# WagnerGroup/pyqmc

Measured on AMD Instinct MI355X. Metric: walker-steps/sec (VMC sweep, 64e- Slater-Jastrow), higher is better.
Workload: dtype f64

## Files before the change

pyqmc_amd/csrc/pqa_capi.hip:

```cpp
#include "pqa_internal.hpp"

static thread_local std::string g_create_error;


static int member_masks(pqa_handle* h, const pqa_system_t* sys, PbcDev& P) {
  P.memb_mask = nullptr;
  P.memb_E = 0;
  const int side = 2 * sys->member_M + 1, E = side, T = side + 2 * E, nc = sys->n_member_class, nj = std::min(sys->nL, 128);
  if ((size_t)nc * T * T * T * 16 > ((size_t)64 << 20)) return 0;
  std::vector<unsigned char> mem((size_t)nc * side * side * side);
  std::vector<int> imgn((size_t)sys->nL * 3);
  HIPCHK(hipMemcpy(mem.data(), sys->member, mem.size(), hipMemcpyDefault));
  HIPCHK(hipMemcpy(imgn.data(), sys->img_n, imgn.size() * sizeof(int), hipMemcpyDefault));
  for (int j = 0; j < nj; ++j)
    for (int c = 0; c < 3; ++c)
      if (std::abs(imgn[3 * j + c]) > E) return 0;
  std::vector<unsigned long long> mask((size_t)nc * T * T * T * 2, 0ull);
  for (int cl = 0; cl < nc; ++cl)
    for (int i0 = 0; i0 < T; ++i0)
      for (int i1 = 0; i1 < T; ++i1)
        for (int i2 = 0; i2 < T; ++i2) {
          unsigned long long* m = &mask[2 * ((((size_t)cl * T + i0) * T + i1) * T + i2)];
          for (int j = 0; j < nj; ++j) {
            const int n0 = i0 - E + imgn[3 * j], n1 = i1 - E + imgn[3 * j + 1], n2 = i2 - E + imgn[3 * j + 2];
// ... 697 lines not shown
        }
        rc2[k] = rc * rc;
      }
      TRY(upload_table(h, rc2.data(), rc2.size(), &tmp_d)); S.ecp_rc2 = tmp_d;
    }
  }
  {
    std::vector<double> quad, quadw;
    ecp_quadrature_tables(quad, quadw);
    TRY(upload_table(h, quad.data(), quad.size(), &h->d_quad));
    TRY(upload_table(h, quadw.data(), quadw.size(), &h->d_quadw));
    std::vector<int> na((size_t)std::max(h->necp, 1), 0), qo((size_t)std::max(h->necp, 1), 0);
    h->ecp_nch.assign((size_t)h->necp, 0);
    for (int k = 0; k < h->necp; ++k) {
      h->ecp_nch[k] = sys->ecp_chan_off[k + 1] - sys->ecp_chan_off[k];
      na[k] = h->ecp_nch[k] <= 2 ? 6 : 12;
      qo[k] = ecp_quadrature_offset(na[k]);
    }
    TRY(upload_table(h, na.data(), na.size(), &h->d_ecp_naip));
    TRY(upload_table(h, qo.data(), qo.size(), &h->d_ecp_qoff));
    S.ecp_naip = h->d_ecp_naip; S.ecp_qoff = h->d_ecp_qoff;
    S.ecp_naip_max = 0;
    for (int k = 0; k < h->necp; ++k) S.ecp_naip_max = std::max(S.ecp_naip_max, na[k]);
  }
  {
    std::vector<int> ptk, pti;
    for (int k = 0; k < h->necp; ++k) {
      const int nch = sys->ecp_chan_off[k + 1] - sys->ecp_chan_off[k];
      const int naip = nch <= 2 ? 6 : 12;
      for (int i = 0; i < naip; ++i) { ptk.push_back(k); pti.push_back(i); }
    }
    h->tm_P = (int)ptk.size();
    TRY(upload_table(h, ptk.data(), ptk.size(), &h->d_ptk));
    TRY(upload_table(h, pti.data(), pti.size(), &h->d_pti));
  }
  return 0;
}

extern "C" int pqa_create(const pqa_system_t* sys, int device, pqa_handle_t** out) {
  *out = nullptr;
  pqa_handle* h = new pqa_handle();
  h->device = device;
  int rc = create_impl(h, sys);
  if (rc) {
    g_create_error = h->err;
    pqa_destroy(h);
    return rc;
  }
  *out = h;
  return 0;
}

extern "C" void pqa_destroy(pqa_handle_t* h) {
  if (!h) return;
  (void)hipSetDevice(h->device);
  if (h->stream) (void)hipStreamSynchronize(h->stream);
  for (void* p : h->owned) (void)hipFree(p);
  DevBuf* bufs[] = {&h->b_x, &h->b_T[0], &h->b_T[1], &h->b_dsign[0], &h->b_dsign[1], &h->b_dlog[0], &h->b_dlog[1],
                    &h->b_cache[0], &h->b_cache[1], &h->b_aval, &h->b_bval, &h->b_pts, &h->b_motmp, &h->b_out, &h->b_widx,
                    &h->b_mask, &h->b_ao, &h->b_flag, &h->b_newpos, &h->b_aux, &h->b_accept, &h->b_accrec, &h->b_acccnt, &h->b_accw,
                    &h->b_gauss, &h->b_unif, &h->b_kc, &h->b_en, &h->b_means, &h->b_sign, &h->b_log, &h->b_ju, &h->b_rot,
                    &h->b_eunif, &h->b_elocal, &h->b_ecnt, &h->b_eoff, &h->b_epts[0], &h->b_epts[1], &h->b_ewgt[0],
                    &h->b_ewgt[1], &h->b_epte[0], &h->b_epte[1], &h->b_emo[0], &h->b_emo[1], &h->b_ecp, &h->b_xt, &h->b_Tt[0], &h->b_Tt[1], &h->b_rc[0], &h->b_rc[1], &h->b_sel[0], &h->b_sel[1], &h->b_auxt, &h->b_kpart, &h->b_rbuf, &h->b_vbuf, &h->b_act, &h->b_alt_x, &h->b_alt_T[0], &h->b_alt_T[1], &h->b_alt_dsign[0], &h->b_alt_dsign[1], &h->b_alt_dlog[0], &h->b_alt_dlog[1], &h->b_alt_cache[0], &h->b_alt_cache[1], &h->b_alt_aval, &h->b_alt_bval, &h->b_alt_j3u, &h->b_rsidx, &h->b_tpos, &h->b_twgt, &h->b_tlive, &h->b_trat, &h->b_tmcnt, &h->b_tmoff, &h->b_tmpass, &h->b_tmamp, &h->b_tmacc, &h->b_tmidx, &h->b_tmapos, &h->b_tmu, &h->b_tmtile, &h->b_tmaoff, &h->b_tmptw, &h->b_tmmarks, &h->b_dmcw, &h->b_dmcold, &h->b_dmcr2, &h->b_dmcout, &h->b_j3u, &h->b_dwrap, &h->b_wrap, &h->b_epass, &h->b_eptw[0], &h->b_eptw[1], &h->b_econ[0], &h->b_econ[1], &h->b_eu0[0], &h->b_eu0[1], &h->b_tves, &h->b_pgdet, &h->b_pbcd0, &h->b_pbcmask, &h->b_pbcth, &h->b_tmuold, &h->b_gauss_b, &h->b_unif_b, &h->b_orbphi[0], &h->b_orbphi[1], &h->b_s2out, &h->b_symx, &h->b_symdet[0], &h->b_symdet[1], &h->b_symout, &h->b_sqq, &h->b_sqout, &h->b_sqpart, &h->b_sqacc, &h->b_e2tab, &h->b_e2out, &h->b_e2acc};
  for (DevBuf* b : bufs)
    if (b->p) (void)hipFree(b->p);
  for (auto& d : h->dm)
    for (DevBuf* b : {&d.pos, &d.row, &d.f, &d.newpos, &d.keep_pos, &d.keep_row, &d.keep_f, &d.cfg})
      if (b->p) (void)hipFree(b->p);
  for (DevBuf* b : {&h->dm_val, &h->dm_norm[0], &h->dm_norm[1], &h->dm_tmp, &h->dm_ijkl, &h->dm_assign[0], &h->dm_assign[1], &h->dm_ratio, &h->dm_acc})
    if (b->p) (void)hipFree(b->p);
  for (auto& pr : h->prof_events) { (void)hipEventDestroy(pr.first); (void)hipEventDestroy(pr.second); }
  for (auto& pr : h->prof2_events) { (void)hipEventDestroy(pr.first); (void)hipEventDestroy(pr.second); }
  for (auto& pr : h->prof3_events) { (void)hipEventDestroy(pr.first); (void)hipEventDestroy(pr.second); }
  if (h->ev0) (void)hipEventDestroy(h->ev0);
  if (h->ev1) (void)hipEventDestroy(h->ev1);
  if (h->pin_tot) (void)hipHostFree(h->pin_tot);
  if (h->b_ovl.p) (void)hipFree(h->b_ovl.p);
  if (h->pin_ovl) (void)hipHostFree(h->pin_ovl);
  if (h->en_stream) { (void)hipStreamSynchronize(h->en_stream); (void)hipStreamDestroy(h->en_stream); }
  if (h->draw_stream) { (void)hipStreamSynchronize(h->draw_stream); (void)hipStreamDestroy(h->draw_stream); }
  for (hipEvent_t e : h->draw_ev) if (e) (void)hipEventDestroy(e);
  for (hipEvent_t e : h->en_ev)
    if (e) (void)hipEventDestroy(e);
  if (h->stream) (void)hipStreamDestroy(h->stream);
  delete h;
}
// ... 98 lines not shown
  } else
    FAIL("unknown parameter name");
  h->saved_valid = false;
  return 0;
}

extern "C" int pqa_get_param(pqa_handle_t* h, const char* name, double* out, int64_t n) {
  HIPCHK(hipSetDevice(h->device));
  HIPCHK(hipStreamSynchronize(h->stream));
  const std::string k(name);
  const double* src = nullptr;
  int64_t want = 0;
  if (k == "acoeff") { src = h->d_acoeff; want = (int64_t)h->natom * h->na * 2; }
  else if (k == "bcoeff") { src = h->d_bcoeff; want = (int64_t)h->nb * 3; }
  else if (k == "det_coeff") { src = h->d_detcoeff; want = h->ndet; }
  else if (k == "mo_coeff_alpha") { src = h->d_mo[0]; want = (int64_t)h->nao * h->nmo[0]; }
  else if (k == "mo_coeff_beta") { src = h->d_mo[1]; want = (int64_t)h->nao * h->nmo[1]; }
  else if (k == "radial_table_info") {
    if (n != 2) FAIL("parameter size mismatch");
    long used = 0;
    for (size_t q = 0; q + 1 < h->rt_shells.size(); q += 2)
      if (h->rt_shells[q] >= 0) used = std::max(used, (long)h->rt_shells[q] + (long)h->rt_shells[q + 1] * PQA_RT_REC);
    out[0] = (double)used; out[1] = h->rt_err;
    return 0;
  }
  else FAIL("unknown parameter name");
  if (n != want) FAIL("parameter size mismatch");
  HIPCHK(hipMemcpy(out, src, n * sizeof(double), hipMemcpyDefault));
  return 0;
}


extern "C" int pqa_eval_ao(pqa_handle_t* h, const double* pts, int64_t npts, int ncomp, double* out) {
  HIPCHK(hipSetDevice(h->device));
  if (!h->has_slater) FAIL("handle has no orbital tables");
  if (ncomp != 1 && ncomp != 4 && ncomp != 5) FAIL("ncomp must be 1, 4 or 5");
  if (h->twist) FAIL("AO-only evaluation is not available for twisted cells (complex AOs); use pqa_eval_mo");
  if (npts <= 0) return 0;
  const size_t nout = (size_t)ncomp * npts * h->nao;
  TRY(ensure(h, h->b_pts, (size_t)npts * 3 * sizeof(double)));
  TRY(ensure(h, h->b_ao, nout * sizeof(double)));
  TRY(copy_in(h, h->b_pts.p, pts, (size_t)npts * 3 * sizeof(double)));
  const dim3 grid((unsigned)((npts + 63) / 64)), block(64);
  TRY(launch_ao(h, plain_points((const double*)h->b_pts.p, npts), npts, ncomp, (double*)h->b_ao.p));
  TRY(check_launch(h, "k_ao"));
  return copy_out(h, out, h->b_ao.p, nout * sizeof(double));
// ... 1046 lines not shown
  if (launches) *launches = h->prof3_launches;
  if (total_ms) *total_ms = h->prof3_ms;
  if (groups) {
    LwCtx lc;
    TRY(lw_setup(h, false, lc));
    *groups = lc.Gm;
  }
  return 0;
}
extern "C" int pqa_set_ecp_naip(pqa_handle_t* h, int32_t naip) {
  HIPCHK(hipSetDevice(h->device));
  if (naip != 0 && ecp_quadrature_offset(naip) < 0) FAIL("naip must be one of 6, 12, 18, 26, 32, 50 (eval_ecp.py:266-267), or 0 for the per-atom default");
  if (h->necp == 0) { h->ecp_naip = naip; return 0; }
  std::vector<int> na((size_t)h->necp), qo((size_t)h->necp);
  for (int k = 0; k < h->necp; ++k) {
    na[k] = naip ? naip : (h->ecp_nch[k] <= 2 ? 6 : 12);
    qo[k] = ecp_quadrature_offset(na[k]);
  }
  HIPCHK(hipStreamSynchronize(h->stream));
  h->ecp_hint_valid = false; h->last_ecp_dev[0] = h->last_ecp_dev[1] = nullptr;
  if (h->last_ecp_points < 0) h->last_ecp_points = 0;
  h->S.ecp_naip_max = 0;
  for (int k = 0; k < h->necp; ++k) h->S.ecp_naip_max = std::max(h->S.ecp_naip_max, na[k]);
  HIPCHK(hipMemcpy(h->d_ecp_naip, na.data(), na.size() * sizeof(int), hipMemcpyHostToDevice));
  HIPCHK(hipMemcpy(h->d_ecp_qoff, qo.data(), qo.size() * sizeof(int), hipMemcpyHostToDevice));
  h->ecp_naip = naip;
  return 0;
}
extern "C" int pqa_last_ecp_points(pqa_handle_t* h, int64_t* npoints) {
  if (h->last_ecp_points < 0 && h->last_ecp_dev[0]) {
    HIPCHK(hipSetDevice(h->device));
    long t[2];
    TRY(copy_in(h, &t[0], h->last_ecp_dev[0], sizeof(long)));
    TRY(copy_out(h, &t[1], h->last_ecp_dev[1], sizeof(long)));
    h->last_ecp_points = t[0] + t[1];
  }
  *npoints = h->last_ecp_points;
  return 0;
}
```

pyqmc_amd/csrc/pqa_ecp.hpp:

```cpp
#pragma once
#include "pqa_energy.hpp"
#include "pqa_lw.hpp"

#define PQA_ECP_WB 4

struct EcpTab {
  const int* ecp_chan_off;
  const int* ecp_term_off;
  const int* ecp_term_n;
  const double* ecp_term_exp;
  const double* ecp_term_coef;
  const double* atom;
  const int* naip;
  const int* qoff;
};

__host__ __device__ inline size_t ecp_tab_bytes(int necp, int nchan, int nterm) {
  const size_t d = (size_t)4 * necp + 2 * (size_t)nterm, i = (size_t)(necp + 1) + (nchan + 1) + nterm + 2 * (size_t)necp;
  return d * sizeof(double) + ((i + 1) / 2) * 2 * sizeof(int);
}

__device__ __forceinline__ EcpTab ecp_stage(const SysDev& S, int nchan, int nterm, double* lds, int tid, int nthreads) {
  double* atom = lds;
  double* ex = atom + 4 * S.necp;
// ... 207 lines not shown
          const double* qd = B.quad + 3 * (qoff + ip);
          const double vx = Rm[0] * qd[0] + Rm[1] * qd[1] + Rm[2] * qd[2];
          const double vy = Rm[3] * qd[0] + Rm[4] * qd[1] + Rm[5] * qd[2];
          const double vz = Rm[6] * qd[0] + Rm[7] * qd[1] + Rm[8] * qd[2];
          const double rix = r * vx, riy = r * vy, riz = r * vz;
          const double cosv = (dx * rix + dy * riy + dz * riz) / (r * sqrt(rix * rix + riy * riy + riz * riz));
          double wsum = 0.0;
          for (int c = 0; c < nch - 1; ++c) wsum += (v[c] / prob) * (2 * c + 1) * legendre_l(c, cosv);
          const long slot = off + ip;
          B.pts[s][3 * slot] = (x0 - dx) + rix;
          B.pts[s][3 * slot + 1] = (y0 - dy) + riy;
          B.pts[s][3 * slot + 2] = (z0 - dz) + riz;
          B.wgt[s][slot] = wsum * B.quadw[qoff + ip];
          B.pte[s][slot] = e;
          B.ptw[s][slot] = (int)w;
          B.u0[s][slot] = U0;
        }
    }
    __builtin_amdgcn_fence(__ATOMIC_ACQ_REL, "wavefront");
    __builtin_amdgcn_wave_barrier();
  }
}

template <bool PBC, bool CX = false>
static __global__ __launch_bounds__(256) void k_ecp_point_lw(SysDev S, LwState L, EcpBuf B, int s, int has_slater, int has_jastrow,
                                                      const double* __restrict__ mo, long npts, long W, double* __restrict__ contrib,
                                                      const double* __restrict__ mo1 = nullptr, long npts1 = 0, double* __restrict__ contrib1 = nullptr) {
  if (blockIdx.y) { s = 1; mo = mo1; npts = npts1; contrib = contrib1; }
  const long p = (long)blockIdx.x * 256 + threadIdx.x;
  if (p >= npts || (B.ptot[s] && p >= *B.ptot[s])) return;
  const int e = B.pte[s][p];
  const long w = B.ptw[s][p];
  const int n = s ? S.ndn : S.nup, i = e - s * S.nup, nmo = S.nmo[s];
  double ratio = 1.0, ratio_im = 0.0;
  if (has_slater) {
    const double* row = mo + (size_t)p * nmo;
    if (CX) {
      const double* Ti = L.Tt[s] + (size_t)i * 2 * n * W + w;
      const int* occ = S.det_occ[s];
      const int nh = nmo / 2;
      double rr = 0.0, ri = 0.0;
      const bool lines = S.occ_ident[s] && ((n | nh) & 7) == 0;
      for (int k0 = 0; k0 < n; k0 += 8) {
        double tr[8], ti[8], a[8], b[8];
#pragma unroll
        for (int u = 0; u < 8; ++u) {
          const int k = (k0 + u < n) ? k0 + u : n - 1;
          tr[u] = Ti[(size_t)(2 * k) * W]; ti[u] = Ti[(size_t)(2 * k + 1) * W];
        }
        if (lines) {
          const double4 al = *reinterpret_cast<const double4*>(row + k0), ah = *reinterpret_cast<const double4*>(row + k0 + 4);
          const double4 bl = *reinterpret_cast<const double4*>(row + nh + k0), bh = *reinterpret_cast<const double4*>(row + nh + k0 + 4);
          a[0] = al.x; a[1] = al.y; a[2] = al.z; a[3] = al.w; a[4] = ah.x; a[5] = ah.y; a[6] = ah.z; a[7] = ah.w;
          b[0] = bl.x; b[1] = bl.y; b[2] = bl.z; b[3] = bl.w; b[4] = bh.x; b[5] = bh.y; b[6] = bh.z; b[7] = bh.w;
        } else {
#pragma unroll
          for (int u = 0; u < 8; ++u) {
            const int o = occ[(k0 + u < n) ? k0 + u : n - 1];
// ... 18 lines not shown
        for (int u = 0; u < 16; ++u) t[u] = Ti[(size_t)(k0 + u) * W];
#pragma unroll
        for (int u = 0; u < 4; ++u) {
          r += q[u].x * t[4 * u]; r += q[u].y * t[4 * u + 1]; r += q[u].z * t[4 * u + 2]; r += q[u].w * t[4 * u + 3];
        }
      }
    } else {
      const int* occ = S.det_occ[s];
      for (int k = 0; k < n; ++k) r += row[occ[k]] * Ti[(size_t)k * W];
    }
    ratio = r;
    }
  }
  if (has_jastrow) {
    double U, g[3], lp, ee, ei;
    if (S.jq_on) jas_eval_lane_m<0, PBC, true, true>(S, L.xt, W, w, e, B.pts[s][3 * p], B.pts[s][3 * p + 1], B.pts[s][3 * p + 2], 1, 0, 1, U, g, lp, ee, ei, -1, true);
    else jas_eval_lane<0, PBC>(S, L.xt, W, w, e, B.pts[s][3 * p], B.pts[s][3 * p + 1], B.pts[s][3 * p + 2], 1, 0, 1, U, g, lp, ee, ei);
    const double ej = exp(U - B.u0[s][p]);
    ratio *= ej; ratio_im *= ej;
  }
  contrib[p] = ratio * B.wgt[s][p];
  if (CX) contrib[npts + p] = ratio_im * B.wgt[s][p];
}
```

pyqmc_amd/csrc/pqa_energy.hip:

```cpp
#include "pqa_internal.hpp"

int energy_dev(pqa_handle* h, double threshold, const double* rot, const double* unif, uint64_t seed, uint32_t step,
               bool soa_current, bool aos_T_needed, bool assemble) {
  const long W = h->W;
  struct JsxOnce { pqa_handle* h; ~JsxOnce() { h->jsx_current = false; } } jsx_once{h};
  if (!soa_current) h->jsx_current = false;
  bool soa_T = false;
  struct Side { pqa_handle* h = nullptr; hipStream_t main = nullptr; ~Side() { if (h) h->stream = main; } } side;
  bool side_join = false;
  TRY(ensure(h, h->b_kc, (size_t)4 * W * sizeof(double)));
  TRY(ensure(h, h->b_en, (size_t)(h->cplx ? 7 : 6) * W * sizeof(double)));
  const bool will_defer = h->necp > 0 && h->ecpb_on == 0 && h->ecp_defer != 0 && !h->S.pbc && h->ecp_hint_valid && (h->ecp_evals % 16) != 0 &&
                          (W * (long)h->N * h->necp * std::max(h->S.ecp_naip_max, 1)) * (long)(64 + 8 * std::max(h->nmo[0], h->nmo[1])) <= (long)256 << 20;
  auto side_begin = [&]() -> int {
    if (!h->en_stream) {
      HIPCHK(hipStreamCreateWithFlags(&h->en_stream, hipStreamNonBlocking));
      for (hipEvent_t& e : h->en_ev) HIPCHK(hipEventCreateWithFlags(&e, hipEventDisableTiming));
    }
    HIPCHK(hipEventRecord(h->en_ev[0], h->stream));
    HIPCHK(hipStreamWaitEvent(h->en_stream, h->en_ev[0], 0));
    side.main = h->stream; side.h = h;
    h->stream = h->en_stream;
    return 0;
  };
// ... 50 lines not shown
    hipLaunchKernelGGL((k_ewald<>), dim3((unsigned)W), dim3(PQA_EWALD_T), lds_ew, h->stream, h->S, h->ew, x,
                       soa ? 1L : (long)h->N * 3, soa ? 3 * W : 3L, soa ? W : 1L, W, (double*)h->b_kc.p);
    TRY(check_launch(h, "k_ewald"));
  }
  if (side.h) {
    HIPCHK(hipEventRecord(h->en_ev[1], h->stream));
    h->stream = side.main;
    side.h = nullptr;
    side_join = true;
  }
  const double* d_ecp = nullptr;
  h->last_ecp_points = 0;
  if (h->necp > 0) {
    const size_t nrot = (size_t)h->N * h->necp;
    TRY(ensure(h, h->b_rot, nrot * 9 * sizeof(double)));
    if (rot) TRY(copy_in(h, h->b_rot.p, rot, nrot * 9 * sizeof(double)));
    else {
      hipLaunchKernelGGL((k_gen_rot<>), dim3((unsigned)((nrot + 63) / 64)), dim3(64), 0, h->stream, (int)nrot, seed, step, (double*)h->b_rot.p);
      TRY(check_launch(h, "k_gen_rot"));
    }
    EcpBuf B{};
    B.rot = (const double*)h->b_rot.p;
    const bool batched = h->ecpb_on != 0;
    if (unif && !batched) {
      TRY(ensure(h, h->b_eunif, nrot * W * sizeof(double)));
      TRY(copy_in(h, h->b_eunif.p, unif, nrot * W * sizeof(double)));
      B.unif = (const double*)h->b_eunif.p;
    }
    B.quad = h->d_quad; B.quadw = h->d_quadw; B.seed = seed; B.step = step; B.threshold = threshold;
    TRY(ensure(h, h->b_elocal, W * sizeof(double)));
    const size_t tab_b = ecp_tab_bytes(h->necp, h->ecp_nchan, h->ecp_nterm);
    const bool ecp_t = h->ecp_lds && h->necp <= 64 && (long)h->necp * ((h->N + 63) / 64) <= 64 && tab_b <= 32768;
    const long nseg = (!batched && ecp_t && h->S.pbc) ? h->necp : 1, nsw = nseg * W;
    B.nseg = (int)nseg;
    TRY(ensure(h, h->b_ecnt, 2 * nsw * sizeof(int)));
    TRY(ensure(h, h->b_eoff, 2 * (nsw + 1) * sizeof(long)));
    TRY(ensure(h, h->b_ecp, (h->cplx ? 2 : 1) * W * sizeof(double)));
    TRY(ensure(h, h->b_epass, (size_t)W * h->necp * ((h->N + 63) / 64) * sizeof(unsigned long long)));
    B.local = (double*)h->b_elocal.p; B.cnt = (int*)h->b_ecnt.p; B.off = (long*)h->b_eoff.p;
    B.passbits = (unsigned long long*)h->b_epass.p;
    B.has_j2 = h->has_j2 ? 1 : 0;
    B.ue = (soa_current && h->has_j2) ? (const double*)h->b_kpart.p + (size_t)4 * h->N * W : nullptr;
    const dim3 g_t((unsigned)((W + PQA_ECP_WB - 1) / PQA_ECP_WB)), b_t(64 * PQA_ECP_WB);
    long tot[2];
    bool defer = false;
    const long* cnt_dev[2] = {nullptr, nullptr};
// ... 39 lines not shown
          TRY(copy_out(h, mk, h->b_tmmarks.p, 4 * sizeof(long)));
          tot[0] = mk[1]; tot[1] = mk[3];
        }
        h->ecp_hint[0] = tot[0]; h->ecp_hint[1] = tot[1]; h->ecp_hint_valid = true;
      }
      ++h->ecp_evals;
      cnt_dev[0] = B.off + nsw; cnt_dev[1] = B.off + (nsw + 1) + nsw;
      B.ptot[0] = defer ? cnt_dev[0] : nullptr; B.ptot[1] = defer ? cnt_dev[1] : nullptr;
    }
    }
    h->last_ecp_points = defer ? -1 : tot[0] + tot[1];
    h->ecp_last_tot[0] = defer ? -1 : tot[0]; h->ecp_last_tot[1] = defer ? -1 : tot[1]; h->ecp_last_nseg = B.nseg;
    h->last_ecp_dev[0] = defer ? cnt_dev[0] : nullptr; h->last_ecp_dev[1] = defer ? cnt_dev[1] : nullptr;
    for (int s = 0; s < 2; ++s) {
      const size_t n = (size_t)std::max<long>(tot[s], 1);
      TRY(ensure(h, h->b_epts[s], n * 3 * sizeof(double)));
      TRY(ensure(h, h->b_ewgt[s], n * sizeof(double)));
      TRY(ensure(h, h->b_epte[s], n * sizeof(int)));
      TRY(ensure(h, h->b_eptw[s], n * sizeof(int)));
      TRY(ensure(h, h->b_econ[s], (h->cplx ? 2 : 1) * n * sizeof(double)));
      TRY(ensure(h, h->b_eu0[s], n * sizeof(double)));
      B.ptw[s] = (int*)h->b_eptw[s].p;
      B.u0[s] = (double*)h->b_eu0[s].p;
      TRY(ensure(h, h->b_emo[s], n * std::max(h->nmo[s], 1) * sizeof(double)));
      B.pts[s] = (double*)h->b_epts[s].p; B.wgt[s] = (double*)h->b_ewgt[s].p; B.pte[s] = (int*)h->b_epte[s].p;
    }
    if (batched) {
      const dim3 g_b((unsigned)((W + PQA_ECPB_WB - 1) / PQA_ECPB_WB)), b_b(64 * PQA_ECPB_WB);
      if (h->S.pbc) hipLaunchKernelGGL(k_ecpb_fill<true>, g_b, b_b, 0, h->stream, h->S, h->js, B, A, W);
      else hipLaunchKernelGGL(k_ecpb_fill<false>, g_b, b_b, 0, h->stream, h->S, h->js, B, A, W);
      TRY(check_launch(h, "k_ecpb_fill"));
    }
    if (side_join && soa_current) HIPCHK(hipStreamWaitEvent(h->stream, h->en_ev[1], 0));
    if (tot[0] + tot[1] > 0) {
      if (batched) {
      } else
      if (ecp_t) {
        if (B.ue) {
          if (h->S.pbc) hipLaunchKernelGGL((k_ecp_fill_t<true, true>), g_t, b_t, tab_b, h->stream, h->S, h->js, B, h->ecp_nchan, h->ecp_nterm, W);
          else hipLaunchKernelGGL((k_ecp_fill_t<false, true>), g_t, b_t, tab_b, h->stream, h->S, h->js, B, h->ecp_nchan, h->ecp_nterm, W);
        } else {
          if (h->S.pbc) hipLaunchKernelGGL((k_ecp_fill_t<true, false>), g_t, b_t, tab_b, h->stream, h->S, h->js, B, h->ecp_nchan, h->ecp_nterm, W);
          else hipLaunchKernelGGL((k_ecp_fill_t<false, false>), g_t, b_t, tab_b, h->stream, h->S, h->js, B, h->ecp_nchan, h->ecp_nterm, W);
        }
      } else
      if (h->S.pbc) hipLaunchKernelGGL(k_ecp_fill<true>, dim3((unsigned)W), dim3(64), 0, h->stream, h->S, h->js, B, W);
      else hipLaunchKernelGGL(k_ecp_fill<false>, dim3((unsigned)W), dim3(64), 0, h->stream, h->S, h->js, B, W);
      TRY(check_launch(h, "k_ecp_fill"));
      if (h->has_slater)
        for (int s = 0; s < 2; ++s) {
          PointAddr pa = plain_points(B.pts[s], tot[s]);
          if (defer) { pa.count = cnt_dev[s]; h->orb_p_hint = std::max<long>(h->ecp_hint[s], 1); }
          const int rc = launch_orb(h, s, pa, tot[s], 1, (double*)h->b_emo[s].p);
          h->orb_p_hint = 0;
          if (rc != 0) return rc;
        }
    }
    const bool acc4 = h->ecp_acc_waves == 4 || (h->ecp_acc_waves == 0 && W * h->N <= 32768);
#define PQA_ECP_ACC(PB, CXF, SC) do { const size_t st_ = (size_t)(SC) * lds_det(h, 1); const int str_ = (int)(st_ / sizeof(double)); \
      if (acc4) hipLaunchKernelGGL((k_ecp_accum<PB, CXF, 4>), dim3((unsigned)W), dim3(256), 4 * st_, h->stream, h->S, h->st, h->js, B, (int)h->has_slater, \
                                   (int)h->has_jastrow, (const double*)h->b_emo[0].p, (const double*)h->b_emo[1].p, W, (double*)h->b_ecp.p, str_); \
      else hipLaunchKernelGGL((k_ecp_accum<PB, CXF, 1>), dim3((unsigned)W), dim3(64), st_, h->stream, h->S, h->st, h->js, B, (int)h->has_slater, \
                              (int)h->has_jastrow, (const double*)h->b_emo[0].p, (const double*)h->b_emo[1].p, W, (double*)h->b_ecp.p, str_); } while (0)
    const bool cx_points = h->cplx && soa_current && h->ndet == 1 && !h->has_j3 && h->ecp_wave == 0 && h->ecp_point_lw;
    if (h->cplx && !cx_points) {
      if (h->S.pbc) PQA_ECP_ACC(true, true, 2); else PQA_ECP_ACC(false, true, 2);
    } else
    if (h->ndet == 1 && !h->has_j3 && h->ecp_wave == 0) {
      const bool both = (cx_points || (soa_current && !h->cplx && h->ecp_point_lw)) && tot[0] > 0 && tot[1] > 0 &&
                        std::max(h->ecp_hint[0], h->ecp_hint[1]) <= 262144 && h->ecp_hint_valid;
      if (both) {
        const dim3 g2((unsigned)((std::max(tot[0], tot[1]) + 255) / 256), 2);
#define PQA_PT2(PB, CXF) hipLaunchKernelGGL((k_ecp_point_lw<PB, CXF>), g2, dim3(256), 0, h->stream, h->S, lw_state(h), B, 0, (int)h->has_slater, (int)h->has_jastrow, \
                                            (const double*)h->b_emo[0].p, tot[0], W, (double*)h->b_econ[0].p, (const double*)h->b_emo[1].p, tot[1], (double*)h->b_econ[1].p)
        if (cx_points) { if (h->S.pbc) PQA_PT2(true, true); else PQA_PT2(false, true); }
        else { if (h->S.pbc) PQA_PT2(true, false); else PQA_PT2(false, false); }
#undef PQA_PT2
      } else
      for (int s = 0; s < 2; ++s) {
        if (tot[s] <= 0) continue;
        const dim3 g((unsigned)((tot[s] + 255) / 256));
        const long n_s = s ? h->ndn : h->nup;
        const double* Tb = soa_T ? (const double*)h->b_Tt[s].p : (const double*)h->st.T[s];
        const long sw = soa_T ? 1 : n_s * n_s, si = soa_T ? n_s * W : n_s, sk = soa_T ? W : 1;
        if (cx_points) {
          if (h->S.pbc)
            hipLaunchKernelGGL((k_ecp_point_lw<true, true>), g, dim3(256), 0, h->stream, h->S, lw_state(h), B, s, (int)h->has_slater,
                               (int)h->has_jastrow, (const double*)h->b_emo[s].p, tot[s], W, (double*)h->b_econ[s].p);
          else
            hipLaunchKernelGGL((k_ecp_point_lw<false, true>), g, dim3(256), 0, h->stream, h->S, lw_state(h), B, s, (int)h->has_slater,
                               (int)h->has_jastrow, (const double*)h->b_emo[s].p, tot[s], W, (double*)h->b_econ[s].p);
        } else
        if (soa_current && !h->cplx && h->ecp_point_lw) {
          if (h->S.pbc)
            hipLaunchKernelGGL(k_ecp_point_lw<true>, g, dim3(256), 0, h->stream, h->S, lw_state(h), B, s, (int)h->has_slater,
                               (int)h->has_jastrow, (const double*)h->b_emo[s].p, tot[s], W, (double*)h->b_econ[s].p);
          else
            hipLaunchKernelGGL(k_ecp_point_lw<false>, g, dim3(256), 0, h->stream, h->S, lw_state(h), B, s, (int)h->has_slater,
                               (int)h->has_jastrow, (const double*)h->b_emo[s].p, tot[s], W, (double*)h->b_econ[s].p);
        } else
        if (h->S.pbc)
          hipLaunchKernelGGL(k_ecp_point<true>, g, dim3(256), 0, h->stream, h->S, h->st, h->js, B, s, (int)h->has_slater,
                             (int)h->has_jastrow, (const double*)h->b_emo[s].p, tot[s], (double*)h->b_econ[s].p, Tb, sw, si, sk);
        else
          hipLaunchKernelGGL(k_ecp_point<false>, g, dim3(256), 0, h->stream, h->S, h->st, h->js, B, s, (int)h->has_slater,
                             (int)h->has_jastrow, (const double*)h->b_emo[s].p, tot[s], (double*)h->b_econ[s].p, Tb, sw, si, sk);
      }
// ... 138 lines not shown
```

pyqmc_amd/csrc/pqa_energy.hpp:

```cpp
#pragma once
#include "pqa_erfc_tab.hpp"
#include "pqa_common.hpp"
#include "pqa_jastrow.hpp"
#include "pqa_slater.hpp"
#include "pqa_cslater.hpp"

template <bool CX, int NWV = 1>
static __global__ __launch_bounds__(64 * NWV) void k_kinetic_coulomb(SysDev S, SlaterState st, JastrowState js, int has_slater,
                                                              int has_jastrow, long W, double* __restrict__ out, int lds_stride) {
  extern __shared__ double lds_all[];
  __shared__ double wsum[4][NWV];
  const int wv = (NWV > 1) ? __builtin_amdgcn_readfirstlane((int)(threadIdx.x >> 6)) : 0;
  double* lds = lds_all + (size_t)wv * lds_stride;
  const long w = blockIdx.x;
  const int lane = threadIdx.x & 63;
  const double* xw = js.x + (size_t)w * S.nelec * 3;
  double ke = 0.0, grad2 = 0.0;
  for (int eb = 0; eb < S.nelec; eb += NWV) {
    const bool valid = eb + wv < S.nelec;
    const int e = valid ? eb + wv : S.nelec - 1;
    double gs[3] = {0.0, 0.0, 0.0}, ls = 0.0, gsi[3] = {0.0, 0.0, 0.0};
    if (has_slater) {
      const int s = e >= S.nup, i = e - s * S.nup, n = s ? S.ndn : S.nup, nmo = S.nmo[s];
      if (CX) {
// ... 540 lines not shown
  __shared__ double part[256];
  double s = 0.0;
  for (long w = threadIdx.x; w < W; w += 256) {
    double v;
    if (r == 0) v = kc[w];
    else if (r == 1) v = kc[W + w];
    else if (r == 2) v = kc[2 * W + w];
    else if (r == 3) v = ecp ? ecp[w] : 0.0;
    else if (r == 4) v = kc[3 * W + w];
    else if (r == 5) { const double ke = kc[w], ee = kc[W + w], ei = kc[2 * W + w], ec = ecp ? ecp[w] : 0.0; v = ke + ee + ei + ec + ii; }
    else v = ecp ? ecp[W + w] : 0.0;
    out[(size_t)r * W + w] = v;
    s += v;
  }
  part[threadIdx.x] = s;
  __syncthreads();
  for (int off = 128; off > 0; off >>= 1) {
    if ((int)threadIdx.x < off) part[threadIdx.x] += part[threadIdx.x + off];
    __syncthreads();
  }
  if (threadIdx.x == 0) means[r] = part[0] / (double)W;
}

template <bool PBC>
static __global__ __launch_bounds__(256) void k_ecp_point(SysDev S, SlaterState st, JastrowState js, EcpBuf B, int s, int has_slater,
                                                   int has_jastrow, const double* __restrict__ mo, long npts,
                                                   double* __restrict__ contrib, const double* __restrict__ Tbase, long sw, long si, long sk) {
  const long p = (long)blockIdx.x * 256 + threadIdx.x;
  if (p >= npts || (B.ptot[s] && p >= *B.ptot[s])) return;
  const int e = B.pte[s][p];
  const long w = B.ptw[s][p];
  const int n = s ? S.ndn : S.nup, i = e - s * S.nup, nmo = S.nmo[s];
  double ratio = 1.0;
  if (has_slater) {
    const double* Ti = Tbase + (size_t)w * sw + (size_t)i * si;
    const double* row = mo + (size_t)p * nmo;
    const int* occ = S.det_occ[s];
    double r = 0.0;
    if (S.occ_ident[s] && (n % 4) == 0 && (nmo % 4) == 0) {
      const double4* row4 = reinterpret_cast<const double4*>(row);
      for (int k4 = 0; k4 < n / 4; ++k4) {
        const double4 q = row4[k4];
        const double* Tk = Ti + (size_t)(4 * k4) * sk;
        r += q.x * Tk[0]; r += q.y * Tk[sk]; r += q.z * Tk[2 * sk]; r += q.w * Tk[3 * sk];
      }
    } else
      for (int k = 0; k < n; ++k) r += row[occ[k]] * Ti[(size_t)k * sk];
    ratio = r;
  }
  if (has_jastrow) {
    const double* xw = js.x + (size_t)w * S.nelec * 3;
    const double nx = B.pts[s][3 * p], ny = B.pts[s][3 * p + 1], nz = B.pts[s][3 * p + 2];
    const int edown = e >= S.nup;
    const double irb = 1.0 / S.rcut_b, ira = 1.0 / S.rcut_a;
    double du = 0.0;
    auto norm = [&](double dx, double dy, double dz) {
      if (PBC) min_image_j(S, dx, dy, dz);
// ... 159 lines not shown
```

pyqmc_amd/csrc/pqa_internal.hpp:

```cpp
#pragma once
#include <hip/hip_runtime.h>

#include <algorithm>
#include <array>
#include <cmath>
#include <cstdio>
#include <cstdlib>
#include <cstring>
#include <string>
#include <vector>

#include "../../include/pyqmc_amd.h"
#include "pqa_ao.hpp"
#include "pqa_common.hpp"
#include "pqa_cslater.hpp"
#include "pqa_dmc.hpp"
#include "pqa_energy.hpp"
#include "pqa_ecp.hpp"
#include "pqa_ecpb.hpp"
#include "pqa_jastrow.hpp"
#include "pqa_lw.hpp"
#include "pqa_slater.hpp"
#include "pqa_res.hpp"
#include "pqa_res8_tab.hpp"
// ... 50 lines not shown
  ChunkTab tab[2]{};
  const unsigned char* out_sel = nullptr;
  long out_slot_stride = 0;
  int orb_col0 = 0;
  double* d_mo[2] = {nullptr, nullptr};
  double* d_cpad[2][2] = {{nullptr, nullptr}, {nullptr, nullptr}};
  double *d_acoeff = nullptr, *d_bcoeff = nullptr, *d_detcoeff = nullptr, *d_quad = nullptr, *d_quadw = nullptr;
  int *d_ecp_naip = nullptr, *d_ecp_qoff = nullptr;
  int ecp_naip = 0;
  std::vector<int> ecp_nch;
  int ecpb_on = 0, ecpb_npoints = 0, ecpb_nsd = 0, ecpb_nsr = 0, ecpb_nsel = 0;
  int *d_ecpb_naip = nullptr, *d_ecpb_qoff = nullptr, *d_ecpb_pstart = nullptr;
  double *d_aq = nullptr, *d_bq = nullptr;
  int jas_merge = 1;
  long W = 0;
  SlaterState st{};
  JastrowState js{};
  DevBuf b_x, b_T[2], b_dsign[2], b_dlog[2], b_cache[2], b_aval, b_bval;
  DevBuf b_alt_x, b_alt_T[2], b_alt_dsign[2], b_alt_dlog[2], b_alt_cache[2], b_alt_aval, b_alt_bval, b_alt_j3u, b_rsidx;
  DevBuf b_pts, b_motmp, b_out, b_widx, b_mask, b_ao, b_flag, b_newpos, b_aux, b_accept, b_accrec, b_acccnt, b_accw, b_dwrap, b_wrap, b_epass, b_eptw[2], b_econ[2], b_eu0[2], b_tves, b_pgdet, b_pbcd0, b_pbcmask, b_pbcth, b_tmuold;
  int* d_colmap[2] = {nullptr, nullptr};
  int ecp_wave = 0;
  int ecp_point_lw = 1;
  int step_pre = 1;
  int ecp_acc_waves = 0;
  int jas_fold_allowed = 1;
  int ecp_lds = 1;
  int ecp_nchan = 0, ecp_nterm = 0;
  long wrap_W = 0;
  DevBuf b_gauss, b_unif, b_kc, b_en, b_means, b_sign, b_log, b_ju;
  DevBuf b_orbphi[2];
  DevBuf b_s2out;
  DevBuf b_symx, b_symdet[2], b_symout;
  DevBuf b_sqq, b_sqout, b_sqpart, b_sqacc;
  DevBuf b_e2tab, b_e2out, b_e2acc;
  DevBuf b_ovl;
  int* pin_ovl = nullptr;
  DevBuf b_tpos, b_twgt, b_tlive, b_trat;
  DevBuf b_tmcnt, b_tmoff, b_tmpass, b_tmamp, b_tmacc, b_tmidx, b_tmapos, b_tmu, b_tmtile, b_tmaoff, b_tmptw, b_tmmarks, b_dmcw, b_dmcold, b_dmcr2, b_dmcout;
  int tm_P = 0;
  int *d_ptk = nullptr, *d_pti = nullptr;
  DevBuf b_xt, b_Tt[2], b_rc[2], b_sel[2], b_auxt, b_kpart, b_rbuf, b_vbuf, b_act;
  int lw_kb = -1;
  int lw_gm = 0;
  DevBuf b_rot, b_eunif, b_elocal, b_ecnt, b_eoff, b_epts[2], b_ewgt[2], b_epte[2], b_emo[2], b_ecp;
  int orb_tp = 0;
  struct TpTune { float ms[2] = {1e30f, 1e30f}; int n[2] = {0, 0}; int choice = 0; };
  TpTune tp_tune[2][48];
  WideTab wide[2]{};
  std::vector<const void*> wide_attr;
  int orb_ws = -1;
  int res_mode = -1;
  bool res_ready = false, res_ok = false;
  bool res_dense = false;
  int res_rows4 = 0;
  double* d_cres[2] = {nullptr, nullptr};
  ResTab res_tab{};
  size_t res_lds = 0;
  int res_lmax = 0;
  int pbc_mincls = 0;
  bool pbc_lists_ok = false;
  int r8_mode = -1;
  bool r8_ready = false, r8_ok = false;
  R8Tab r8_tab{};
  size_t r8_lds = 0;
  double r8_util = 0.0;
  bool r8_xaos_next = false;
  bool jsx_current = false;
// ... 163 lines not shown
```

Measured before the change: 3.119 million.

## Compute ECP determinant ratios via AO-space vector dot instead of MO evaluation

Adds a kernel that first forms V = C_occ·T for each point's electron column with f64 MFMA in shared memory, then evaluates AO shells at the quadrature point and dots them directly with V. The per-point ratio is stored, so the point kernels can skip materialising full MO rows for every ECP quadrature point. This targets the cost of MO evaluation plus the row·T dot for non-PBC, real, single-determinant ECP energy. It adds a new LDS-heavy kernel with its own eligibility conditions and a diagnostic parameter. The measured metric is a VMC sweep, and the ECP energy step may not dominate it.

Result: faster. 3.188 million, median of 6 (+2.2%).

```diff
diff --git a/pyqmc_amd/csrc/pqa_capi.hip b/pyqmc_amd/csrc/pqa_capi.hip
--- a/pyqmc_amd/csrc/pqa_capi.hip
+++ b/pyqmc_amd/csrc/pqa_capi.hip
@@ -743,6 +743,7 @@
     S.ecp_naip = h->d_ecp_naip; S.ecp_qoff = h->d_ecp_qoff;
     S.ecp_naip_max = 0;
     for (int k = 0; k < h->necp; ++k) S.ecp_naip_max = std::max(S.ecp_naip_max, na[k]);
+    h->ecp_naip_min = h->necp ? *std::min_element(na.begin(), na.end()) : 0;
   }
   {
     std::vector<int> ptk, pti;
@@ -782,7 +783,7 @@
                     &h->b_mask, &h->b_ao, &h->b_flag, &h->b_newpos, &h->b_aux, &h->b_accept, &h->b_accrec, &h->b_acccnt, &h->b_accw,
                     &h->b_gauss, &h->b_unif, &h->b_kc, &h->b_en, &h->b_means, &h->b_sign, &h->b_log, &h->b_ju, &h->b_rot,
                     &h->b_eunif, &h->b_elocal, &h->b_ecnt, &h->b_eoff, &h->b_epts[0], &h->b_epts[1], &h->b_ewgt[0],
-                    &h->b_ewgt[1], &h->b_epte[0], &h->b_epte[1], &h->b_emo[0], &h->b_emo[1], &h->b_ecp, &h->b_xt, &h->b_Tt[0], &h->b_Tt[1], &h->b_rc[0], &h->b_rc[1], &h->b_sel[0], &h->b_sel[1], &h->b_auxt, &h->b_kpart, &h->b_rbuf, &h->b_vbuf, &h->b_act, &h->b_alt_x, &h->b_alt_T[0], &h->b_alt_T[1], &h->b_alt_dsign[0], &h->b_alt_dsign[1], &h->b_alt_dlog[0], &h->b_alt_dlog[1], &h->b_alt_cache[0], &h->b_alt_cache[1], &h->b_alt_aval, &h->b_alt_bval, &h->b_alt_j3u, &h->b_rsidx, &h->b_tpos, &h->b_twgt, &h->b_tlive, &h->b_trat, &h->b_tmcnt, &h->b_tmoff, &h->b_tmpass, &h->b_tmamp, &h->b_tmacc, &h->b_tmidx, &h->b_tmapos, &h->b_tmu, &h->b_tmtile, &h->b_tmaoff, &h->b_tmptw, &h->b_tmmarks, &h->b_dmcw, &h->b_dmcold, &h->b_dmcr2, &h->b_dmcout, &h->b_j3u, &h->b_dwrap, &h->b_wrap, &h->b_epass, &h->b_eptw[0], &h->b_eptw[1], &h->b_econ[0], &h->b_econ[1], &h->b_eu0[0], &h->b_eu0[1], &h->b_tves, &h->b_pgdet, &h->b_pbcd0, &h->b_pbcmask, &h->b_pbcth, &h->b_tmuold, &h->b_gauss_b, &h->b_unif_b, &h->b_orbphi[0], &h->b_orbphi[1], &h->b_s2out, &h->b_symx, &h->b_symdet[0], &h->b_symdet[1], &h->b_symout, &h->b_sqq, &h->b_sqout, &h->b_sqpart, &h->b_sqacc, &h->b_e2tab, &h->b_e2out, &h->b_e2acc};
+                    &h->b_ewgt[1], &h->b_epte[0], &h->b_epte[1], &h->b_emo[0], &h->b_emo[1], &h->b_ecp, &h->b_xt, &h->b_Tt[0], &h->b_Tt[1], &h->b_rc[0], &h->b_rc[1], &h->b_sel[0], &h->b_sel[1], &h->b_auxt, &h->b_kpart, &h->b_rbuf, &h->b_vbuf, &h->b_act, &h->b_alt_x, &h->b_alt_T[0], &h->b_alt_T[1], &h->b_alt_dsign[0], &h->b_alt_dsign[1], &h->b_alt_dlog[0], &h->b_alt_dlog[1], &h->b_alt_cache[0], &h->b_alt_cache[1], &h->b_alt_aval, &h->b_alt_bval, &h->b_alt_j3u, &h->b_rsidx, &h->b_tpos, &h->b_twgt, &h->b_tlive, &h->b_trat, &h->b_tmcnt, &h->b_tmoff, &h->b_tmpass, &h->b_tmamp, &h->b_tmacc, &h->b_tmidx, &h->b_tmapos, &h->b_tmu, &h->b_tmtile, &h->b_tmaoff, &h->b_tmptw, &h->b_tmmarks, &h->b_dmcw, &h->b_dmcold, &h->b_dmcr2, &h->b_dmcout, &h->b_j3u, &h->b_dwrap, &h->b_wrap, &h->b_epass, &h->b_eptw[0], &h->b_eptw[1], &h->b_econ[0], &h->b_econ[1], &h->b_eu0[0], &h->b_eu0[1], &h->b_erat[0], &h->b_erat[1], &h->b_tves, &h->b_pgdet, &h->b_pbcd0, &h->b_pbcmask, &h->b_pbcth, &h->b_tmuold, &h->b_gauss_b, &h->b_unif_b, &h->b_orbphi[0], &h->b_orbphi[1], &h->b_s2out, &h->b_symx, &h->b_symdet[0], &h->b_symdet[1], &h->b_symout, &h->b_sqq, &h->b_sqout, &h->b_sqpart, &h->b_sqacc, &h->b_e2tab, &h->b_e2out, &h->b_e2acc};
   for (DevBuf* b : bufs)
     if (b->p) (void)hipFree(b->p);
   for (auto& d : h->dm)
@@ -927,6 +928,11 @@
     for (size_t q = 0; q + 1 < h->rt_shells.size(); q += 2)
       if (h->rt_shells[q] >= 0) used = std::max(used, (long)h->rt_shells[q] + (long)h->rt_shells[q + 1] * PQA_RT_REC);
     out[0] = (double)used; out[1] = h->rt_err;
+    return 0;
+  }
+  else if (k == "ecp_vec_used") {
+    if (n != 1) FAIL("parameter size mismatch");
+    out[0] = (double)h->ecp_vec_used;
     return 0;
   }
   else FAIL("unknown parameter name");
@@ -2019,6 +2025,7 @@
   if (h->last_ecp_points < 0) h->last_ecp_points = 0;
   h->S.ecp_naip_max = 0;
   for (int k = 0; k < h->necp; ++k) h->S.ecp_naip_max = std::max(h->S.ecp_naip_max, na[k]);
+  h->ecp_naip_min = *std::min_element(na.begin(), na.end());
   HIPCHK(hipMemcpy(h->d_ecp_naip, na.data(), na.size() * sizeof(int), hipMemcpyHostToDevice));
   HIPCHK(hipMemcpy(h->d_ecp_qoff, qo.data(), qo.size() * sizeof(int), hipMemcpyHostToDevice));
   h->ecp_naip = naip;
diff --git a/pyqmc_amd/csrc/pqa_ecp.hpp b/pyqmc_amd/csrc/pqa_ecp.hpp
--- a/pyqmc_amd/csrc/pqa_ecp.hpp
+++ b/pyqmc_amd/csrc/pqa_ecp.hpp
@@ -1,4 +1,5 @@
 #pragma once
+#include "pqa_ao.hpp"
 #include "pqa_energy.hpp"
 #include "pqa_lw.hpp"
 
@@ -253,7 +254,7 @@
   }
 }
 
-template <bool PBC, bool CX = false>
+template <bool PBC, bool CX = false, bool RAT = false>
 static __global__ __launch_bounds__(256) void k_ecp_point_lw(SysDev S, LwState L, EcpBuf B, int s, int has_slater, int has_jastrow,
                                                       const double* __restrict__ mo, long npts, long W, double* __restrict__ contrib,
                                                       const double* __restrict__ mo1 = nullptr, long npts1 = 0, double* __restrict__ contrib1 = nullptr) {
@@ -264,7 +265,8 @@
   const long w = B.ptw[s][p];
   const int n = s ? S.ndn : S.nup, i = e - s * S.nup, nmo = S.nmo[s];
   double ratio = 1.0, ratio_im = 0.0;
-  if (has_slater) {
+  if (has_slater && RAT) ratio = mo[p];
+  else if (has_slater) {
     const double* row = mo + (size_t)p * nmo;
     if (CX) {
       const double* Ti = L.Tt[s] + (size_t)i * 2 * n * W + w;
@@ -329,3 +331,96 @@
   contrib[p] = ratio * B.wgt[s][p];
   if (CX) contrib[npts + p] = ratio_im * B.wgt[s][p];
 }
+
+#define PQA_EV_NC 16
+#define PQA_EV_MINRULE 6
+__host__ __device__ inline int ecp_vecdot_stride(int rows_pad) { return (((rows_pad + 15) / 16) * 16) | 1; }
+__host__ __device__ inline size_t ecp_vecdot_lds(int rows_pad, int n, int nshell, int nprim) {
+  const int n4 = (n + 3) & ~3;
+  const size_t tp = (size_t)n4 * PQA_EV_NC > 256 ? (size_t)n4 * PQA_EV_NC : 256;
+  return ((size_t)PQA_EV_NC * ecp_vecdot_stride(rows_pad) + tp + 3 * (size_t)nshell + 2 * (size_t)nprim) * sizeof(double) +
+         ((size_t)7 * nshell + 128) * sizeof(int);
+}
+template <int PQA_UNIT = 0>
+static __global__ __launch_bounds__(256) void k_ecp_vecdot(SysDev S, ChunkTab T, int spin, PointAddr pa, long P, const int* __restrict__ pte,
+                                                           const int* __restrict__ ptw, const double* __restrict__ Tbase, long sw, long si, long sk,
+                                                           int rows_pad, double* __restrict__ ratio) {
+  P = point_count(pa, P);
+  if ((long)blockIdx.x * 64 >= P) return;
+  extern __shared__ double lds[];
+  const int n = spin ? S.ndn : S.nup, n4 = (n + 3) & ~3, vs = ecp_vecdot_stride(rows_pad);
+  double* Vs = lds;
+  double* Tp = Vs + (size_t)PQA_EV_NC * vs;
+  double* sh_xyz = Tp + (n4 * PQA_EV_NC > 256 ? n4 * PQA_EV_NC : 256);
+  double* pr_exp = sh_xyz + 3 * S.nshell;
+  double* pr_coef = pr_exp + S.nprim;
+  int* sh_meta = reinterpret_cast<int*>(pr_coef + S.nprim);
+  int* own = sh_meta + 7 * S.nshell;
+  const int tid = threadIdx.x, lane = tid & 63, wv = __builtin_amdgcn_readfirstlane(tid >> 6);
+  for (int sh = tid; sh < S.nshell; sh += 256) {
+    const int ia = S.shell_atom[sh];
+    sh_xyz[3 * sh] = S.atom_xyz[3 * ia]; sh_xyz[3 * sh + 1] = S.atom_xyz[3 * ia + 1]; sh_xyz[3 * sh + 2] = S.atom_xyz[3 * ia + 2];
+    int* m = sh_meta + 7 * sh;
+    m[0] = S.shell_l[sh]; m[1] = S.shell_prim_off[sh + 1] - S.shell_prim_off[sh]; m[2] = S.shell_prim_off[sh]; m[3] = T.shell_kb[sh];
+    m[4] = ia; m[5] = S.shell_rt[2 * sh]; m[6] = S.shell_rt[2 * sh + 1];
+  }
+  for (int p = tid; p < S.nprim; p += 256) { pr_exp[p] = S.prim_exp[p]; pr_coef[p] = S.prim_coef[p]; }
+  const long p0 = (long)blockIdx.x * 64;
+  const bool plive = p0 + lane < P;
+  const long pmine = plive ? p0 + lane : P - 1;
+  double px, py, pz;
+  load_point(pa, pmine, px, py, pz);
+  const int pe = pte[pmine], pw = ptw[pmine];
+  int col, ncol;
+  {
+    const int qe = __shfl_up(pe, 1, 64), qw = __shfl_up(pw, 1, 64);
+    const int first = (lane > 0 && (qe != pe || qw != pw)) ? 1 : 0;
+    col = wave_excl_scan(first, lane, ncol) + first;
+    ncol += 1;
+    if (wv == 0 && (first || lane == 0)) { own[2 * col] = pw; own[2 * col + 1] = pe - spin * S.nup; }
+  }
+  const double* __restrict__ C = T.cpad[spin];
+  const int ldc = T.ldc[spin];
+  const int* __restrict__ occ = S.det_occ[spin];
+  const int i16 = lane & 15, kq = lane >> 4;
+  const int* __restrict__ cw_off = T.cw_off[0];
+  const int* __restrict__ cw_shell = T.cw_shell[0];
+  __syncthreads();
+  {
+    for (int idx = tid; idx < n4 * PQA_EV_NC; idx += 256) {
+      const int k = idx / PQA_EV_NC, c = idx % PQA_EV_NC;
+      Tp[idx] = (k < n && c < ncol) ? Tbase[(size_t)own[2 * c] * sw + (size_t)own[2 * c + 1] * si + (size_t)k * sk] : 0.0;
+    }
+    __syncthreads();
+    for (int rt = wv; rt * 16 < rows_pad; rt += 4) {
+      d4 acc = (d4){0.0, 0.0, 0.0, 0.0};
+      const double* crow = C + (size_t)(16 * rt + i16) * ldc;
+      for (int k0 = 0; k0 < n4; k0 += 4) {
+        const int k = k0 + kq;
+        const double a = crow[occ[k < n ? k : n - 1]];
+        acc = __builtin_amdgcn_mfma_f64_16x16x4f64(a, Tp[k * PQA_EV_NC + i16], acc, 0, 0, 0);
+      }
+#pragma unroll
+      for (int r = 0; r < 4; ++r) Vs[(size_t)i16 * vs + 16 * rt + kq + 4 * r] = acc[r];
+    }
+    __syncthreads();
+    const double* __restrict__ Vc = Vs + (size_t)(col < PQA_EV_NC ? col : PQA_EV_NC - 1) * vs;
+    double dot = 0.0;
+    for (int ch = 0; ch < T.nchunk; ++ch) {
+      const double* __restrict__ Vr = Vc + T.chunk_row0[ch];
+      const int s_end = cw_off[ch * 4 + wv + 1];
+      for (int q = cw_off[ch * 4 + wv]; q < s_end; ++q) {
+        const int sh = cw_shell[q];
+        const int* m = sh_meta + 7 * sh;
+        const int l_ = m[0], np_ = m[1], q0 = m[2], kb = m[3], rt_ = m[5], rn_ = m[6];
+        const double x = px - sh_xyz[3 * sh], y = py - sh_xyz[3 * sh + 1], z = pz - sh_xyz[3 * sh + 2];
+        auto to_dot = [&](int mm, double v, double, double, double, double) { dot = fma(v, Vr[kb + mm], dot); };
+        if (rt_ >= 0) shell_eval_tab(l_, x, y, z, S.rtab + rt_, rn_, to_dot);
+        else shell_eval<1>(l_, x, y, z, pr_exp + q0, pr_coef + q0, np_, to_dot);
+      }
+    }
+    Tp[wv * 64 + lane] = dot;
+    __syncthreads();
+    if (wv == 0 && plive) ratio[p0 + lane] = ((Tp[lane] + Tp[64 + lane]) + Tp[128 + lane]) + Tp[192 + lane];
+  }
+}
diff --git a/pyqmc_amd/csrc/pqa_energy.hip b/pyqmc_amd/csrc/pqa_energy.hip
--- a/pyqmc_amd/csrc/pqa_energy.hip
+++ b/pyqmc_amd/csrc/pqa_energy.hip
@@ -96,6 +96,10 @@
     EcpBuf B{};
     B.rot = (const double*)h->b_rot.p;
     const bool batched = h->ecpb_on != 0;
+    const int vec_rows = h->chunks[1].rows_pad;
+    const size_t vec_lds = ecp_vecdot_lds(vec_rows, std::max(h->nup, h->ndn), h->nshell, (int)h->S.nprim);
+    const bool vec = !batched && h->has_slater && !h->cplx && !h->S.pbc && h->ndet == 1 && !h->has_j3 && h->ecp_wave == 0 && h->ecp_point_lw &&
+                     !h->big && vec_lds <= (size_t)64 * 1024 && h->ecp_naip_min >= PQA_EV_MINRULE;
     if (unif && !batched) {
       TRY(ensure(h, h->b_eunif, nrot * W * sizeof(double)));
       TRY(copy_in(h, h->b_eunif.p, unif, nrot * W * sizeof(double)));
@@ -181,7 +185,9 @@
       TRY(ensure(h, h->b_eu0[s], n * sizeof(double)));
       B.ptw[s] = (int*)h->b_eptw[s].p;
       B.u0[s] = (double*)h->b_eu0[s].p;
-      TRY(ensure(h, h->b_emo[s], n * std::max(h->nmo[s], 1) * sizeof(double)));
+      h->ecp_vec_used = vec ? 1 : 0;
+      if (vec) TRY(ensure(h, h->b_erat[s], n * sizeof(double)));
+      else TRY(ensure(h, h->b_emo[s], n * std::max(h->nmo[s], 1) * sizeof(double)));
       B.pts[s] = (double*)h->b_epts[s].p; B.wgt[s] = (double*)h->b_ewgt[s].p; B.pte[s] = (int*)h->b_epte[s].p;
     }
     if (batched) {
@@ -206,6 +212,19 @@
       if (h->S.pbc) hipLaunchKernelGGL(k_ecp_fill<true>, dim3((unsigned)W), dim3(64), 0, h->stream, h->S, h->js, B, W);
       else hipLaunchKernelGGL(k_ecp_fill<false>, dim3((unsigned)W), dim3(64), 0, h->stream, h->S, h->js, B, W);
       TRY(check_launch(h, "k_ecp_fill"));
+      if (vec) {
+        for (int s = 0; s < 2; ++s) {
+          if (tot[s] <= 0) continue;
+          PointAddr pa = plain_points(B.pts[s], tot[s]);
+          if (defer) pa.count = cnt_dev[s];
+          const long n_s = s ? h->ndn : h->nup;
+          const double* Tb = soa_current ? (const double*)h->b_Tt[s].p : (const double*)h->st.T[s];
+          const long sw = soa_current ? 1 : n_s * n_s, si = soa_current ? n_s * W : n_s, sk = soa_current ? W : 1;
+          hipLaunchKernelGGL((k_ecp_vecdot<>), dim3((unsigned)((tot[s] + 63) / 64)), dim3(256), vec_lds, h->stream, h->S, h->tab[1], s, pa, tot[s],
+                             (const int*)B.pte[s], (const int*)B.ptw[s], Tb, sw, si, sk, vec_rows, (double*)h->b_erat[s].p);
+        }
+        TRY(check_launch(h, "k_ecp_vecdot"));
+      } else
       if (h->has_slater)
         for (int s = 0; s < 2; ++s) {
           PointAddr pa = plain_points(B.pts[s], tot[s]);
@@ -232,7 +251,10 @@
         const dim3 g2((unsigned)((std::max(tot[0], tot[1]) + 255) / 256), 2);
 #define PQA_PT2(PB, CXF) hipLaunchKernelGGL((k_ecp_point_lw<PB, CXF>), g2, dim3(256), 0, h->stream, h->S, lw_state(h), B, 0, (int)h->has_slater, (int)h->has_jastrow, \
                                             (const double*)h->b_emo[0].p, tot[0], W, (double*)h->b_econ[0].p, (const double*)h->b_emo[1].p, tot[1], (double*)h->b_econ[1].p)
-        if (cx_points) { if (h->S.pbc) PQA_PT2(true, true); else PQA_PT2(false, true); }
+        if (vec)
+          hipLaunchKernelGGL((k_ecp_point_lw<false, false, true>), g2, dim3(256), 0, h->stream, h->S, lw_state(h), B, 0, 1, (int)h->has_jastrow,
+                             (const double*)h->b_erat[0].p, tot[0], W, (double*)h->b_econ[0].p, (const double*)h->b_erat[1].p, tot[1], (double*)h->b_econ[1].p);
+        else if (cx_points) { if (h->S.pbc) PQA_PT2(true, true); else PQA_PT2(false, true); }
         else { if (h->S.pbc) PQA_PT2(true, false); else PQA_PT2(false, false); }
 #undef PQA_PT2
       } else
@@ -242,6 +264,14 @@
         const long n_s = s ? h->ndn : h->nup;
         const double* Tb = soa_T ? (const double*)h->b_Tt[s].p : (const double*)h->st.T[s];
         const long sw = soa_T ? 1 : n_s * n_s, si = soa_T ? n_s * W : n_s, sk = soa_T ? W : 1;
+        if (vec) {
+          if (soa_current)
+            hipLaunchKernelGGL((k_ecp_point_lw<false, false, true>), g, dim3(256), 0, h->stream, h->S, lw_state(h), B, s, 1, (int)h->has_jastrow,
+                               (const double*)h->b_erat[s].p, tot[s], W, (double*)h->b_econ[s].p);
+          else
+            hipLaunchKernelGGL((k_ecp_point<false, true>), g, dim3(256), 0, h->stream, h->S, h->st, h->js, B, s, 1, (int)h->has_jastrow,
+                               (const double*)h->b_erat[s].p, tot[s], (double*)h->b_econ[s].p, Tb, sw, si, sk);
+        } else
         if (cx_points) {
           if (h->S.pbc)
             hipLaunchKernelGGL((k_ecp_point_lw<true, true>), g, dim3(256), 0, h->stream, h->S, lw_state(h), B, s, (int)h->has_slater,
diff --git a/pyqmc_amd/csrc/pqa_energy.hpp b/pyqmc_amd/csrc/pqa_energy.hpp
--- a/pyqmc_amd/csrc/pqa_energy.hpp
+++ b/pyqmc_amd/csrc/pqa_energy.hpp
@@ -586,7 +586,7 @@
   if (threadIdx.x == 0) means[r] = part[0] / (double)W;
 }
 
-template <bool PBC>
+template <bool PBC, bool RAT = false>
 static __global__ __launch_bounds__(256) void k_ecp_point(SysDev S, SlaterState st, JastrowState js, EcpBuf B, int s, int has_slater,
                                                    int has_jastrow, const double* __restrict__ mo, long npts,
                                                    double* __restrict__ contrib, const double* __restrict__ Tbase, long sw, long si, long sk) {
@@ -596,7 +596,8 @@
   const long w = B.ptw[s][p];
   const int n = s ? S.ndn : S.nup, i = e - s * S.nup, nmo = S.nmo[s];
   double ratio = 1.0;
-  if (has_slater) {
+  if (has_slater && RAT) ratio = mo[p];
+  else if (has_slater) {
     const double* Ti = Tbase + (size_t)w * sw + (size_t)i * si;
     const double* row = mo + (size_t)p * nmo;
     const int* occ = S.det_occ[s];
diff --git a/pyqmc_amd/csrc/pqa_internal.hpp b/pyqmc_amd/csrc/pqa_internal.hpp
--- a/pyqmc_amd/csrc/pqa_internal.hpp
+++ b/pyqmc_amd/csrc/pqa_internal.hpp
@@ -96,6 +96,8 @@
   int* d_colmap[2] = {nullptr, nullptr};
   int ecp_wave = 0;
   int ecp_point_lw = 1;
+  int ecp_naip_min = 0;
+  int ecp_vec_used = 0;
   int step_pre = 1;
   int ecp_acc_waves = 0;
   int jas_fold_allowed = 1;
@@ -118,6 +120,7 @@
   int lw_kb = -1;
   int lw_gm = 0;
   DevBuf b_rot, b_eunif, b_elocal, b_ecnt, b_eoff, b_epts[2], b_ewgt[2], b_epte[2], b_emo[2], b_ecp;
+  DevBuf b_erat[2];
   int orb_tp = 0;
   struct TpTune { float ms[2] = {1e30f, 1e30f}; int n[2] = {0, 0}; int choice = 0; };
   TpTune tp_tune[2][48];
```
